# wengflow/robust-e-nerf

Measured on AMD Instinct MI355X. Metric: train_rays_per_sec, higher is better.
Workload: dtype f32; 1 GPU; BASELINE configs[1]: synthetic ficus-like event stream, 65536 events/step/GPU = 2 renders x 65536 rays x 128 samples, arch ngp, fp32, l_diff (2 renders), fwd+bwd+Adam; sampler=uniform; sampler=uniform, samples_per_ray=128, parallelism=dp1, front_prefetched=False, mlp_precision=highest, device_counts=False, device_count_overflows=0, fwd_chunks=8, dist_world_size=1

## Files before the change

include/ren_amd.h:

```cpp
#ifndef REN_AMD_H
#define REN_AMD_H

#include <stdint.h>

#ifdef __cplusplus
extern "C" {
#endif

typedef enum ren_status {
    REN_OK = 0,
    REN_ERR_BAD_ARG = -1,
    REN_ERR_UNSUPPORTED = -2,
    REN_ERR_LAUNCH = -3
} ren_status;

enum { REN_CT_AABB = 0, REN_CT_TANH = 1, REN_CT_SPHERE = 2 };

#define REN_MAX_LEVELS 16

typedef struct ren_grid_desc {
    int32_t  n_levels;
    float    scale[REN_MAX_LEVELS];
    uint32_t res[REN_MAX_LEVELS];
    uint32_t size[REN_MAX_LEVELS];
    uint32_t offset[REN_MAX_LEVELS];
    uint32_t hashed[REN_MAX_LEVELS];
} ren_grid_desc;

typedef struct ren_scene_desc {
    float   aabb[6];
    int32_t contraction_type;
} ren_scene_desc;


int ren_abi_version(void);
enum { REN_KNOB_HGB_NO_PAIRS = 0, REN_KNOB_HGB_HALVE_REGIONS = 1, REN_KNOB_MARCH_SEQUENTIAL = 2, REN_KNOB_HG_VARIANT = 3,
       REN_KNOB_VFIELD_PLAIN = 4, REN_KNOB_HGB_SUBREGION = 5, REN_KNOB_COUNT = 6 };
int ren_set_knob(int32_t knob, int32_t value);
int ren_get_knob(int32_t knob);
const char *ren_build_info(void);

int ren_trajectory_fwd(const double *ts, int64_t B, const int64_t *tab_ts, const float *tab_pos,
                       const float *tab_quat, int64_t C, float *pos, float *rot, void *stream);
int ren_raygen_fwd(const float *Kinv, const float *px, const float *pos, const float *rot,
                   int64_t B, float *rays_o, float *rays_d, void *stream);
int ren_pose_rays_fwd(const double *ts, int64_t R, const float *px, int64_t px_rows, const float *Kinv,
                      const int64_t *tab_ts, const float *tab_pos, const float *tab_quat, int64_t C,
                      float *rays_o, float *rays_d, void *stream);

int ren_ray_aabb_intersect(const float *rays_o, const float *rays_d, int64_t n_rays,
                           const float *aabb_host, float near_plane, float far_plane,
                           float *t_min, float *t_max, void *stream);
#define REN_MARCH_VERIFIED_DIV 0x100
int ren_ray_march(const float *rays_o, const float *rays_d, const float *t_min,
                  const float *t_max, const float *jitter, int64_t n_rays,
                  const float *roi_host, const int32_t *res_host, const uint8_t *binary,
                  int32_t contraction_type, float step_size, float cone_angle,
                  int32_t mode, int32_t n_uniform,
                  const int64_t *offsets, int32_t *counts,
                  int32_t *ray_indices, float *t_starts, float *t_ends, float *interval_cache,
                  int32_t cache_cap, void *stream);

int ren_march_div_check(const float *roi, int64_t *mismatches, void *stream);
int ren_uniform(uint64_t seed, uint64_t offset, int64_t n, float *out, void *stream);
int ren_exclusive_scan(const int32_t *counts, int64_t n, int64_t *offsets, int64_t *total,
                       int64_t *scratch1024 , void *stream);

int ren_count_guard(int32_t *counts, int32_t *counts_also, int64_t n_rays, const int64_t *total, int64_t capacity,
                    int64_t *n_out, int64_t *stats, void *stream);
int ren_scan_guard(int32_t *counts, int32_t *counts_also, int64_t n_rays, int64_t *offsets, int64_t *total, int64_t capacity,
                   int64_t *n_out, int64_t *stats, int64_t *scratch1024, void *stream);
int ren_frag_zero_tail(float *feat, int64_t capacity, const int64_t *n_dev, void *stream);

int ren_visibility(const int64_t *offsets, const int32_t *counts, int64_t n_rays,
                   const float *sigmas, const float *t_starts, const float *t_ends,
                   float early_stop_eps, float alpha_thre, uint8_t *keep, int32_t *kept_counts,
                   void *stream);
int ren_compact_samples(const int64_t *offsets, const int32_t *counts, const int64_t *new_offsets,
                        int64_t n_rays, const uint8_t *keep, const float *t_starts,
                        const float *t_ends, int32_t *out_ray_indices, float *out_t_starts,
                        float *out_t_ends, void *stream);
int ren_compact_features(const int64_t *offsets, const int32_t *counts, const int64_t *new_offsets, int64_t n_rays,
                         const uint8_t *keep, const float *feat_in, float *feat_out, void *stream);
int ren_pack_info(const int32_t *ray_indices, int64_t n, int64_t n_rays, int64_t *offsets,
                  int32_t *counts, void *stream);

int ren_hashgrid_fwd(const ren_grid_desc *grid, const float *table, const float *x_unit,
                     const ren_scene_desc *scene, const float *rays_o, const float *rays_d,
                     const int32_t *ray_indices, const float *t_starts, const float *t_ends,
                     int64_t n, int32_t layout, float *feat, const int64_t *n_dev, void *stream);
int ren_hashgrid_bwd(const ren_grid_desc *grid, float *grad_table, const float *x_unit,
                     const ren_scene_desc *scene, const float *rays_o, const float *rays_d,
// ... 329 lines not shown
```

robust_e_nerf_amd/_lib.py:

```python
from __future__ import annotations

import ctypes
import os
from ctypes import POINTER, Structure, c_char_p, c_double, c_float, c_int, c_int32, c_int64, c_uint32, c_void_p

HERE = os.path.dirname(os.path.abspath(__file__))
LIB_PATH = os.path.join(HERE, "csrc", "libren_amd.so")
MAX_LEVELS = 16

REN_OK, REN_ERR_BAD_ARG, REN_ERR_UNSUPPORTED, REN_ERR_LAUNCH = 0, -1, -2, -3


class RenError(RuntimeError):
    pass


class GridDesc(Structure):
    _fields_ = [("n_levels", c_int32), ("scale", c_float * MAX_LEVELS), ("res", c_uint32 * MAX_LEVELS),
                ("size", c_uint32 * MAX_LEVELS), ("offset", c_uint32 * MAX_LEVELS),
                ("hashed", c_uint32 * MAX_LEVELS)]


class SceneDesc(Structure):
    _fields_ = [("aabb", c_float * 6), ("contraction_type", c_int32)]


P = c_void_p
SIGNATURES = {
    "ren_abi_version": (c_int, []),
    "ren_build_info": (c_char_p, []),
    "ren_set_knob": (c_int, [c_int32, c_int32]),
    "ren_get_knob": (c_int, [c_int32]),
    "ren_trajectory_fwd": (c_int, [P, c_int64, P, P, P, c_int64, P, P, P]),
    "ren_raygen_fwd": (c_int, [P, P, P, P, c_int64, P, P, P]),
    "ren_pose_rays_fwd": (c_int, [P, c_int64, P, c_int64, P, P, P, P, c_int64, P, P, P]),
    "ren_ray_aabb_intersect": (c_int, [P, P, c_int64, POINTER(c_float), c_float, c_float, P, P, P]),
    "ren_march_div_check": (c_int, [POINTER(c_float), P, P]),
    "ren_ray_march": (c_int, [P, P, P, P, P, c_int64, POINTER(c_float), POINTER(c_int32), P, c_int32,
                              c_float, c_float, c_int32, c_int32, P, P, P, P, P, P, c_int32, P]),
    "ren_compact_features": (c_int, [P, P, P, c_int64, P, P, P, P]),
    "ren_uniform": (c_int, [ctypes.c_uint64, ctypes.c_uint64, c_int64, P, P]),
    "ren_exclusive_scan": (c_int, [P, c_int64, P, P, P, P]),
    "ren_count_guard": (c_int, [P, P, c_int64, P, c_int64, P, P, P]),
    "ren_scan_guard": (c_int, [P, P, c_int64, P, P, c_int64, P, P, P, P]),
    "ren_frag_zero_tail": (c_int, [P, c_int64, P, P]),
    "ren_visibility": (c_int, [P, P, c_int64, P, P, P, c_float, c_float, P, P, P]),
    "ren_compact_samples": (c_int, [P, P, P, c_int64, P, P, P, P, P, P, P]),
    "ren_pack_info": (c_int, [P, c_int64, c_int64, P, P, P]),
    "ren_hashgrid_fwd": (c_int, [POINTER(GridDesc), P, P, POINTER(SceneDesc), P, P, P, P, P, c_int64, c_int32, P, P, P]),
    "ren_hashgrid_bwd": (c_int, [POINTER(GridDesc), P, P, POINTER(SceneDesc), P, P, P, P, P, c_int64, c_int32, P, P]),
    "ren_hashgrid_bwd_input": (c_int, [POINTER(GridDesc), P, P, POINTER(SceneDesc), P, P, P, P, P, c_int64, c_int32, P, P, P]),
    "ren_hashgrid_bwd_binned_workspace_bytes": (c_int64, [c_int64]),
    "ren_hashgrid_bwd_binned": (c_int, [POINTER(GridDesc), P, P, POINTER(SceneDesc), P, P, P, P, P, c_int64, c_int32, P, P, P, P]),
    "ren_hashgrid_bwd_binned_begin": (c_int, [POINTER(GridDesc), P, POINTER(SceneDesc), P, P, P, P, P, c_int64, c_int32, P, P]),
    "ren_hashgrid_bwd_binned_scatter": (c_int, [POINTER(GridDesc), P, P, POINTER(SceneDesc), P, P, P, P, P, c_int64, c_int32, P,
                                                c_int64, c_int64, P, P]),
    "ren_hashgrid_bwd_binned_finish": (c_int, [POINTER(GridDesc), P, c_int64, c_int32, P, P]),
    "ren_mlp_fwd": (c_int, [P, c_int32, c_int32, P, POINTER(SceneDesc), P, P, P, P, P, P, P, c_int64, c_int32, P, P, P, P]),
    "ren_mlp_bwd_workspace_floats": (c_int64, [c_int32]),
    "ren_mlp_bwd": (c_int, [P, c_int32, c_int32, P, P, POINTER(SceneDesc), P, P, P, P, P, P, P, c_int64, P, P, P, P, P, P, P, P]),
    "ren_mlp_fwd_bf16": (c_int, [P, c_int32, c_int32, P, POINTER(SceneDesc), P, P, P, P, P, P, P, c_int64, c_int32, P, P, P, P]),
    "ren_mlp_bwd_bf16": (c_int, [P, c_int32, c_int32, P, P, POINTER(SceneDesc), P, P, P, P, P, P, P, c_int64, P, P, P, P, P, P, P, P]),
    "ren_mlp_act_save_floats": (c_int64, [c_int64]),
    "ren_mlp_fwd_save": (c_int, [P, c_int32, c_int32, c_int32, P, POINTER(SceneDesc), P, P, P, P, P, P, P, c_int64, P, P, P, P, P]),
    "ren_mlp_bwd_saved": (c_int, [P, c_int32, c_int32, c_int32, P, P, P, POINTER(SceneDesc), P, P, P, P, P, P, P, c_int64, P, P, P,
                                  P, P, P, P, P]),
    "ren_act_jvp_fwd": (c_int, [P, c_int32, P, c_int32, c_float, P, c_int32, c_int64, c_int32, P]),
    "ren_act_jvp_bwd": (c_int, [P, P, P, c_int32, P, c_float, P, P, c_int64, c_int32, P]),
    "ren_event_prepare": (c_int, [P, P, P, P, P, P, P, c_int64, c_float, c_float, c_double, P, P, P, P, P, P, P, P, P, P]),
    "ren_event_params_refresh": (c_int, [P, c_float, P, c_double, P, P]),
    "ren_tau_adam_step": (c_int, [P, P, P, c_double, c_double, c_double, c_double, c_double, c_int64, c_double, P]),
    "ren_event_param_grad": (c_int, [c_int32, c_int32, c_int32, P, P, P, P, P, P, P, c_int64, c_float, c_float, c_float,
                                     c_double, c_float, P, P, P, P]),
    "ren_mlp_fwd_x": (c_int, [P, c_int32, c_int32, c_int32, P, POINTER(SceneDesc), P, P, P, P, P, P, P, c_int64, c_int32, P, P, P, P, P, P]),
    "ren_mlp_bwd_x_workspace_floats": (c_int64, [c_int32]),
    "ren_mlp_bwd_x": (c_int, [P, c_int32, c_int32, c_int32, P, P, P, POINTER(SceneDesc), P, P, P, P, P, P, P, c_int64, P, P, P, P, P,
                              P, P, c_int32, P, P]),
    "ren_composite_fwd": (c_int, [P, P, c_int64, P, P, P, P, c_int32, P, P, P, P, P, P, P]),
    "ren_composite_bwd": (c_int, [P, P, c_int64, P, P, P, P, c_int32, P, P, P, P, P, P, P, P, P, P, P, P]),
    "ren_event_loss_fwd": (c_int, [P, P, P, P, c_int64, c_int32, P, P]),
    "ren_event_loss_bwd": (c_int, [P, P, P, P, c_int64, c_int32, c_float, P, P, P, P]),
    "ren_event_diff_loss_fwd": (c_int, [P, P, P, c_int32, c_float, P, c_int32, c_int64, c_int32, P, P]),
    "ren_event_diff_loss_bwd": (c_int, [P, P, P, c_int32, c_float, P, c_int32, c_int64, c_int32, c_float, P, P, P, P, P, P, P, P]),
    "ren_bkgd_param_fwd": (c_int, [P, c_int32, P, P]),
    "ren_bkgd_param_grad": (c_int, [P, c_int64, c_int32, P, P, P, P]),
# ... 109 lines not shown
```

robust_e_nerf_amd/csrc/ren_api.hip:

```cpp
#include "ren_common.h"
extern "C" int ren_abi_version(void) { return 25; }
extern "C" const char *ren_build_info(void) { return "ren_amd gfx950 (CDNA4) hipcc " __VERSION__; }

extern "C" int ren_set_knob(int32_t knob, int32_t value) {
    if (knob < 0 || knob >= REN_KNOB_COUNT) return REN_ERR_BAD_ARG;
    ren_knob_store()[knob].store(value, std::memory_order_relaxed);
    return REN_OK;
}
extern "C" int ren_get_knob(int32_t knob) { return knob < 0 || knob >= REN_KNOB_COUNT ? REN_ERR_BAD_ARG : ren_knob(knob); }
```

robust_e_nerf_amd/csrc/ren_common.h:

```cpp
#pragma once
#include <hip/hip_runtime.h>
#include <stdint.h>
#include <math.h>
#include <stdio.h>
#include "../../include/ren_amd.h"

#define REN_WAVE 64

#undef hipLaunchKernelGGL
#define hipLaunchKernelGGL(kernel, grid, block, shmem, stream, ...)            \
    do {                                                                        \
        (void)hipGetLastError();                                                \
        kernel<<<(grid), (block), (shmem), (stream)>>>(__VA_ARGS__);            \
    } while (0)

#define REN_CHECK_LAUNCH()                                   \
    do {                                                     \
        hipError_t e__ = hipGetLastError();                  \
        if (e__ != hipSuccess)                               \
            fprintf(stderr, "[ren_amd] %s:%d launch error: %s\n", __FILE__, __LINE__, hipGetErrorString(e__)); \
        return e__ == hipSuccess ? REN_OK : REN_ERR_LAUNCH;  \
    } while (0)

static inline int ren_blocks(int64_t n, int threads) { return (int)((n + threads - 1) / threads); }

#include <atomic>
#include <cstdlib>
inline std::atomic<int> *ren_knob_store() {
    static std::atomic<int> knobs[REN_KNOB_COUNT];
    static const bool init = [] {
        const char *names[REN_KNOB_COUNT] = {"REN_HGB_NO_PAIRS", "REN_HGB_HALVE_REGIONS", "REN_MARCH_SEQUENTIAL", "REN_HG_VARIANT",
                                           "REN_VFIELD_PLAIN", "REN_HGB_SUBREGION"};
        const int defaults[REN_KNOB_COUNT] = {0, 0, 0, 2, 0, 1};
        for (int k = 0; k < REN_KNOB_COUNT; ++k) {
            const char *e = getenv(names[k]);
            knobs[k].store(e ? atoi(e) : defaults[k], std::memory_order_relaxed);
        }
        return true;
    }();
    (void)init;
    return knobs;
}
static inline int ren_knob(int k) { return ren_knob_store()[k].load(std::memory_order_relaxed); }

struct ren_scene_dev {
    float lo[3], inv_ext[3];
    float hi[3];
    int ct;
};

static inline ren_scene_dev ren_make_scene(const ren_scene_desc *s) {
    ren_scene_dev d;
    for (int k = 0; k < 3; ++k) {
        d.lo[k] = s->aabb[k];
        d.hi[k] = s->aabb[3 + k];
        d.inv_ext[k] = 1.0f / (s->aabb[3 + k] - s->aabb[k]);
    }
    d.ct = s->contraction_type;
    return d;
}

__device__ __forceinline__ void ren_contract(const ren_scene_dev &sc, float x, float y, float z,
                                             float &ux, float &uy, float &uz) {
    ux = (x - sc.lo[0]) / (sc.hi[0] - sc.lo[0]);
    uy = (y - sc.lo[1]) / (sc.hi[1] - sc.lo[1]);
    uz = (z - sc.lo[2]) / (sc.hi[2] - sc.lo[2]);
    if (sc.ct == REN_CT_SPHERE) {
        ux = ux * 2.f - 1.f; uy = uy * 2.f - 1.f; uz = uz * 2.f - 1.f;
        float mag = sqrtf(ux * ux + uy * uy + uz * uz);
        if (mag > 1.f) {
            float s = (2.f - 1.f / mag) / mag;
            ux *= s; uy *= s; uz *= s;
        }
        ux = ux * 0.25f + 0.5f; uy = uy * 0.25f + 0.5f; uz = uz * 0.25f + 0.5f;
    } else if (sc.ct == REN_CT_TANH) {
        ux = (tanhf(ux - 0.5f) + 1.f) * 0.5f;
        uy = (tanhf(uy - 0.5f) + 1.f) * 0.5f;
        uz = (tanhf(uz - 0.5f) + 1.f) * 0.5f;
    }
}

__device__ __forceinline__ void ren_sample_pos(const float *__restrict__ rays_o,
                                               const float *__restrict__ rays_d,
                                               const int32_t *__restrict__ ray_indices,
                                               const float *__restrict__ t_starts,
                                               const float *__restrict__ t_ends, int64_t i,
                                               float &x, float &y, float &z, int &ray) {
    ray = ray_indices[i];
// ... 19 lines not shown
```

robust_e_nerf_amd/csrc/ren_hashgrid_binned.hip:

```cpp
#include <cstdlib>
#include "ren_hashgrid_common.h"

namespace {

constexpr int BIN_SHIFT = 13;
constexpr int BIN_ENTRIES = 1 << BIN_SHIFT;
constexpr int MAX_BINS_PER_LEVEL = 64;
constexpr int MAX_BINS = REN_MAX_LEVELS * MAX_BINS_PER_LEVEL;
#ifndef REN_SC_THREADS
#define REN_SC_THREADS 512
#endif
#ifndef REN_SC_WAVES
#define REN_SC_WAVES 6
#endif
#ifndef REN_SC_WAVES_PAIR
#define REN_SC_WAVES_PAIR 8
#endif
constexpr int SC_THREADS = REN_SC_THREADS;
constexpr int SC_ENTRIES = SC_THREADS * 8;
constexpr int CNT_THREADS = 1024, CNT_SAMPLES = 1024;
constexpr int64_t PART_ENTRIES_MIN = 1 << 16, PART_ENTRIES_MAX = 1 << 23;
constexpr int N_SUB = 8;
__device__ __forceinline__ int xcd_id() {
    unsigned x;
    asm volatile("s_getreg_b32 %0, hwreg(HW_REG_XCC_ID)" : "=s"(x));
    return (int)(x & (N_SUB - 1));
}
inline int64_t part_entries_for(int64_t n, int64_t hashed_cap) {
    int64_t p = hashed_cap;
    if (p == 0) {
        p = PART_ENTRIES_MIN;
        while (p < (1 << 21) && p * 1024 < n * 128) p <<= 1;
    }
    return p < PART_ENTRIES_MIN ? PART_ENTRIES_MIN : (p > PART_ENTRIES_MAX ? PART_ENTRIES_MAX : p);
}
constexpr int LMAX_SLOTS = 8, LMAX_STRIDE = 32;
constexpr int LMAX_WORDS = REN_MAX_LEVELS * LMAX_SLOTS * LMAX_STRIDE;

struct BinTab {
    int bin_base[REN_MAX_LEVELS + 1];
    uint32_t cap[REN_MAX_LEVELS];
    uint32_t pair[REN_MAX_LEVELS];
    uint32_t skip[REN_MAX_LEVELS];
    int sub_by_xcd;
    int cnt_stride;
    int halve;
};

struct Part {
    uint32_t gbin, single;
    uint64_t begin, end;
};

struct Workspace {
    uint32_t *counts, *level_max, *cursors, *n_parts;
    uint32_t *bin_cap;
    uint64_t *bin_start;
    Part *parts;
    char *pool;
};
constexpr int PAIR_BIN_SHIFT = 26;

struct TanSrc {
    const float *rays_do, *rays_dd, *dfeatd;
};

__device__ __forceinline__ void lds_barrier() { asm volatile("s_waitcnt lgkmcnt(0)\n\ts_barrier" ::: "memory"); }

struct SampleArgs {
    int layout;
    const float *dfeat, *x_unit;
    ren_scene_dev sc;
// ... 122 lines not shown
template <bool TAN>
__global__ __launch_bounds__(CNT_THREADS) void bin_count_kernel(GridDev g, BinTab bt, SampleArgs a,
                                                                uint32_t *__restrict__ counts) {
    __shared__ uint32_t hist[MAX_BINS];
    for (int t = threadIdx.x; t < MAX_BINS; t += CNT_THREADS) hist[t] = 0;
    __syncthreads();
    const int lane = threadIdx.x & 63;
#pragma unroll 1
    for (int k = 0; k < CNT_SAMPLES / CNT_THREADS; ++k) {
        const int64_t i = (int64_t)blockIdx.x * bt.cnt_stride * CNT_SAMPLES + k * CNT_THREADS + threadIdx.x;
        const bool inb = i < ren_eff_n(a.n, a.n_dev);
        float u[3] = {0.f, 0.f, 0.f}, ud[3];
        if (inb) unit_pos<TAN>(a, i, u, ud);
#pragma unroll 1
        for (int lvl = 0; lvl < g.n_levels; ++lvl) {
            if (bt.cap[lvl] || bt.skip[lvl]) continue;
            float d0, d1, e0, e1;
            const bool have = inb && (a.dfeat == nullptr || load_dfeat<TAN>(a, g.n_levels, lvl, i, d0, d1, e0, e1));
            const LevelPos p = level_pos(u[0], u[1], u[2], g.scale[lvl]);
            const uint32_t res = g.res[lvl], size = g.size[lvl];
            const bool hashed = g.hashed[lvl] != 0;
            bool head;
            uint32_t idx[8];
            corner_indices8(p.c[0], p.c[1], p.c[2], res, size, hashed, idx);
            const bool emit = run_tail(!hashed, have, idx[0], lane, head);
#pragma unroll
            for (int c = 0; c < 8; ++c) (void)bin_rank(!hashed, emit, idx[c] >> BIN_SHIFT, lane, hist + lvl * MAX_BINS_PER_LEVEL);
        }
    }
    __syncthreads();
    for (int t = threadIdx.x; t < MAX_BINS; t += CNT_THREADS) {
        const int lvl = t / MAX_BINS_PER_LEVEL, bin = t % MAX_BINS_PER_LEVEL;
        if (lvl < g.n_levels && bin < bt.bin_base[lvl + 1] - bt.bin_base[lvl] && hist[t])
            atomicAdd(&counts[bt.bin_base[lvl] + bin], hist[t]);
    }
}

__global__ __launch_bounds__(MAX_BINS) void bin_offsets_kernel(int n_bins, BinTab bt, uint64_t capacity_slots,
                                                               const uint32_t *__restrict__ counts,
                                                               uint32_t *__restrict__ cursors,
                                                               uint32_t *__restrict__ bin_cap,
                                                               uint64_t *__restrict__ bin_start) {
    __shared__ uint64_t s_cnt[MAX_BINS];
    const int t = threadIdx.x;
    uint64_t c = 0, slots = 0;
    bool pair = false;
    if (t < n_bins) {
        int lvl = 0;
        while (lvl + 1 < REN_MAX_LEVELS && t >= bt.bin_base[lvl + 1]) ++lvl;
        pair = bt.pair[lvl] != 0;
        c = bt.skip[lvl] ? 0 : bt.cap[lvl] ? bt.cap[lvl] : counts[t];
        if (!bt.skip[lvl] && !bt.cap[lvl] && bt.cnt_stride > 1) c = c * bt.cnt_stride + c * bt.cnt_stride / 4 + 4096;
        if (bt.halve) c = c / 2;
        c &= ~(uint64_t)7;
        if (pair) c = (c / N_SUB) & ~(uint64_t)7;
        slots = pair ? c * N_SUB : (c * 10 + 15) / 16;
        for (int x = 0; x < N_SUB; ++x) cursors[t * N_SUB + x] = 0;
    }
    s_cnt[t] = slots;
    __syncthreads();
    for (int off = 1; off < MAX_BINS; off <<= 1) {
        const uint64_t a = t >= off ? s_cnt[t - off] : 0;
        __syncthreads();
        s_cnt[t] += a;
        __syncthreads();
    }
    if (t < n_bins) {
        const uint64_t start = s_cnt[t] - slots;
        uint64_t room = start < capacity_slots ? capacity_slots - start : 0;
        if (room > slots) room = slots;
        if (room < slots) c = (pair ? room / N_SUB : room * 16 / 10) & ~(uint64_t)7;
        bin_start[t] = start < capacity_slots ? start : capacity_slots;
        bin_cap[t] = (uint32_t)c;
    }
    if (t == n_bins - 1) bin_start[n_bins] = s_cnt[t] < capacity_slots ? s_cnt[t] : capacity_slots;
}

__global__ __launch_bounds__(MAX_BINS) void bin_partition_kernel(int n_bins, uint64_t PART_ENTRIES, BinTab bt,
                                                                 const uint32_t *__restrict__ cursors,
                                                                 const uint32_t *__restrict__ bin_cap,
                                                                 Part *__restrict__ parts, uint32_t *__restrict__ n_parts) {
    __shared__ uint32_t s_np[MAX_BINS];
    const int t = threadIdx.x;
    uint64_t c = 0;
    bool pair = false;
    if (t < n_bins) {
        int lvl = 0;
        while (lvl + 1 < REN_MAX_LEVELS && t >= bt.bin_base[lvl + 1]) ++lvl;
        pair = bt.pair[lvl] != 0;
        for (int x = 0; x < (pair ? N_SUB : 1); ++x) c += cursors[t * N_SUB + x] < bin_cap[t] ? cursors[t * N_SUB + x] : bin_cap[t];
    }
    const uint32_t np = pair ? (c ? 1u : 0u) : (uint32_t)((c + PART_ENTRIES - 1) / PART_ENTRIES);
    s_np[t] = np;
    __syncthreads();
    for (int off = 1; off < MAX_BINS; off <<= 1) {
        const uint32_t b = t >= off ? s_np[t - off] : 0;
        __syncthreads();
        s_np[t] += b;
        __syncthreads();
    }
    if (t == n_bins - 1) n_parts[0] = s_np[t];
    const uint32_t pbase = s_np[t] - np;
    for (uint32_t k = 0; k < np; ++k) {
        Part p;
        p.gbin = t; p.single = np == 1;
        p.begin = (uint64_t)k * PART_ENTRIES;
        p.end = k + 1 == np ? c : p.begin + PART_ENTRIES;
        parts[pbase + k] = p;
    }
}

__device__ __forceinline__ void table_atomic(float *grad_table, uint32_t offset, uint32_t idx, float a, float b) {
    float *gt = grad_table + 2 * ((size_t)offset + idx);
    atomicAdd(gt, a);
    atomicAdd(gt + 1, b);
}

template <bool TAN, int KIND>
__global__ __launch_bounds__(SC_THREADS, KIND == 1 ? REN_SC_WAVES_PAIR : REN_SC_WAVES) void bin_scatter_kernel(
    GridDev g, BinTab bt, SampleArgs a, Workspace ws, float *__restrict__ grad_table) {
    __shared__ uint32_t hist[MAX_BINS_PER_LEVEL], loc[MAX_BINS_PER_LEVEL + 1], fit[MAX_BINS_PER_LEVEL];
    __shared__ char *gp0[MAX_BINS_PER_LEVEL], *gp1[MAX_BINS_PER_LEVEL];
    __shared__ __attribute__((aligned(16))) unsigned char stage[KIND == 1 ? SC_THREADS * 4 * 16 : SC_ENTRIES * 12];
    __shared__ float wave_max[SC_THREADS / 64];
    __shared__ int any_overflow;
    uint32_t *st_key = reinterpret_cast<uint32_t *>(stage);
    float2 *st_v = reinterpret_cast<float2 *>(stage + SC_ENTRIES * 4);
    float4 *st_p = reinterpret_cast<float4 *>(stage);
    const int64_t chunk = blockIdx.x;
    const int tid = threadIdx.x, lane = tid & 63;
    const int64_t i = chunk * SC_THREADS + tid;
    const bool inb = i < ren_eff_n(a.n, a.n_dev);
    float u[3] = {0.f, 0.f, 0.f}, ud[3] = {0.f, 0.f, 0.f};
    if (inb) unit_pos<TAN>(a, i, u, ud);
    constexpr bool pairs = KIND == 1;
    const int sub = !pairs ? 0 : bt.sub_by_xcd ? xcd_id() : (int)((chunk >> 3) & (N_SUB - 1));
#pragma unroll 1
    for (int lvl = 0; lvl < g.n_levels; ++lvl) {
        if (bt.skip[lvl]) continue;
        if (KIND == 1 && !bt.pair[lvl]) continue;
        if (KIND == 2 && bt.pair[lvl]) continue;
        if (tid < MAX_BINS_PER_LEVEL) hist[tid] = 0;
        if (tid == 0) any_overflow = 0;
        lds_barrier();
        const uint32_t res = g.res[lvl], size = g.size[lvl];
        const bool hashed = g.hashed[lvl] != 0;
        const float scale = g.scale[lvl];
        float d0 = 0.f, d1 = 0.f, e0 = 0.f, e1 = 0.f;
        const bool valid = inb && load_dfeat<TAN>(a, g.n_levels, lvl, i, d0, d1, e0, e1);
        const LevelPos p = level_pos(u[0], u[1], u[2], scale);
        const float wx1 = p.w[0], wy1 = p.w[1], wz1 = p.w[2], wx0 = 1.f - wx1, wy0 = 1.f - wy1, wz0 = 1.f - wz1;
        if (!valid) { d0 = 0.f; d1 = 0.f; e0 = 0.f; e1 = 0.f; }
        uint32_t key[8];
        float v0[8], v1[8];
        bool have;
        float vmax = 0.f;
        uint32_t idx[8];
        corner_indices8(p.c[0], p.c[1], p.c[2], res, size, hashed, idx);
        if (pairs) {
            const bool same = ((idx[0] ^ idx[1]) >> BIN_SHIFT) == 0;
#pragma unroll
            for (int j = 0; j < 4; ++j) {
                const float wyz = ((j & 1) ? wy1 : wy0) * ((j & 2) ? wz1 : wz0);
                v0[j] = wyz * d0; v1[j] = wyz * d1;
            }
            if (valid && !same) {
#pragma unroll
                for (int j = 0; j < 4; ++j) {
                    table_atomic(grad_table, g.offset[lvl], idx[2 * j], wx0 * v0[j], wx0 * v1[j]);
                    table_atomic(grad_table, g.offset[lvl], idx[2 * j + 1], wx1 * v0[j], wx1 * v1[j]);
                }
            }
            have = valid && same;
// ... 84 lines not shown
            gp0[tid] = q0; gp1[tid] = q1;
        }
        lds_barrier();
        if (have) {
            if (pairs) {
#pragma unroll
                for (int j = 0; j < 4; ++j)
                    st_p[loc[key[j] >> PAIR_BIN_SHIFT] + key[4 + j]] = make_float4(__uint_as_float(key[j]), v0[j], v1[j], wx1);
            } else {
#pragma unroll
                for (int c = 0; c < 8; ++c) {
                    const uint32_t ix = key[c] & 0x7FFFFu;
                    const uint32_t pos = loc[ix >> BIN_SHIFT] + (key[c] >> 19);
                    st_key[pos] = ix;
                    st_v[pos] = make_float2(v0[c], v1[c]);
                }
            }
        }
        lds_barrier();
        const uint32_t total = loc[MAX_BINS_PER_LEVEL];
        const bool ovf = any_overflow != 0;
        if (pairs) {
            for (uint32_t q = tid; q < total; q += SC_THREADS) {
                const float4 r = st_p[q];
                const uint32_t code = __float_as_uint(r.x), b = code >> PAIR_BIN_SHIFT;
                if (!ovf || q - loc[b] < fit[b]) {
                    reinterpret_cast<float4 *>(gp0[b])[q] = r;
                } else {
                    const uint32_t i0 = (b << BIN_SHIFT) | (code & (BIN_ENTRIES - 1));
                    const uint32_t i1 = (b << BIN_SHIFT) | ((code >> BIN_SHIFT) & (BIN_ENTRIES - 1));
                    table_atomic(grad_table, g.offset[lvl], i0, (1.f - r.w) * r.y, (1.f - r.w) * r.z);
                    table_atomic(grad_table, g.offset[lvl], i1, r.w * r.y, r.w * r.z);
                }
            }
            continue;
        }
        for (uint32_t q = tid; q < total; q += SC_THREADS) {
            const uint32_t ix = st_key[q], b = ix >> BIN_SHIFT;
            const float2 v = st_v[q];
            if (!ovf || q - loc[b] < fit[b]) {
                reinterpret_cast<uint16_t *>(gp1[b])[q] = (uint16_t)(ix & (BIN_ENTRIES - 1));
                reinterpret_cast<float2 *>(gp0[b])[q] = v;
            } else {
                table_atomic(grad_table, g.offset[lvl], ix, v.x, v.y);
            }
        }
    }
}

__device__ __forceinline__ long long to_fixed(float v, double scale) {
    return __double2ll_rn((double)v * scale);
}

__global__ __launch_bounds__(1024) void bin_accumulate_kernel(GridDev g, BinTab bt, Workspace ws,
                                                              float *__restrict__ grad_table) {
    extern __shared__ __attribute__((aligned(16))) unsigned long long acc[];
    if (blockIdx.x >= ws.n_parts[0]) return;
    const Part part = ws.parts[blockIdx.x];
    unsigned long long *acc0 = acc, *acc1 = acc + BIN_ENTRIES;
    for (int e = threadIdx.x; e < 2 * BIN_ENTRIES; e += 1024) acc[e] = 0ull;
    int lvl = 0;
    while (lvl + 1 < g.n_levels && (int)part.gbin >= bt.bin_base[lvl + 1]) ++lvl;
    int ex;
    uint32_t lmax = 0;
    for (int k = 0; k < LMAX_SLOTS; ++k) lmax = max(lmax, ws.level_max[(lvl * LMAX_SLOTS + k) * LMAX_STRIDE]);
    (void)frexpf(__uint_as_float(lmax), &ex);
    const double scale = ldexp(1.0, 38 - ex), inv_scale = ldexp(1.0, ex - 38);
    const char *base = ws.pool + ws.bin_start[part.gbin] * 16;
    const uint32_t first = ((uint32_t)part.gbin - bt.bin_base[lvl]) << BIN_SHIFT;
    const uint32_t lim = g.size[lvl] > first ? g.size[lvl] - first : 0;
    float2 *gt = reinterpret_cast<float2 *>(grad_table) + g.offset[lvl] + first;
    constexpr int FL = BIN_ENTRIES / 1024;
    float2 gv[FL];
#pragma unroll
    for (int u = 0; u < FL; ++u) {
        const uint32_t k = threadIdx.x + u * 1024;
        gv[u] = (part.single && k < lim) ? gt[k] : make_float2(0.f, 0.f);
    }
    __syncthreads();
    uint64_t e = part.begin + threadIdx.x;
    if (bt.pair[lvl]) {
        const float4 *rec = reinterpret_cast<const float4 *>(base);
        auto add = [&](const float4 &r) {
            const uint32_t code = __float_as_uint(r.x);
            const uint32_t i0 = code & (BIN_ENTRIES - 1), i1 = (code >> BIN_SHIFT) & (BIN_ENTRIES - 1);
            const float f0 = 1.f - r.w;
            atomicAdd(&acc0[i0], (unsigned long long)to_fixed(f0 * r.y, scale));
            atomicAdd(&acc1[i0], (unsigned long long)to_fixed(f0 * r.z, scale));
            atomicAdd(&acc0[i1], (unsigned long long)to_fixed(r.w * r.y, scale));
            atomicAdd(&acc1[i1], (unsigned long long)to_fixed(r.w * r.z, scale));
        };
        const uint32_t cap = ws.bin_cap[part.gbin];
        for (int x = 0; x < N_SUB; ++x) {
            const float4 *rx = rec + (size_t)x * cap;
            const uint32_t fill = ws.cursors[part.gbin * N_SUB + x];
            const uint64_t end = fill < cap ? fill : cap;
            uint64_t q = threadIdx.x;
            for (; q + 3 * 1024 < end; q += 4 * 1024) {
                float4 r[4];
#pragma unroll
                for (int u = 0; u < 4; ++u) r[u] = rx[q + u * 1024];
#pragma unroll
                for (int u = 0; u < 4; ++u) add(r[u]);
            }
            for (; q < end; q += 1024) add(rx[q]);
        }
    } else {
// ... 6 lines not shown
#pragma unroll
            for (int u = 0; u < 4; ++u) {
                atomicAdd(&acc0[ix[u]], (unsigned long long)to_fixed(v[u].x, scale));
                atomicAdd(&acc1[ix[u]], (unsigned long long)to_fixed(v[u].y, scale));
            }
        }
        for (; e < part.end; e += 1024) {
            const uint32_t idx = out_idx[e];
            const float2 v = out_v[e];
            atomicAdd(&acc0[idx], (unsigned long long)to_fixed(v.x, scale));
            atomicAdd(&acc1[idx], (unsigned long long)to_fixed(v.y, scale));
        }
    }
    __syncthreads();
#pragma unroll
    for (int u = 0; u < FL; ++u) {
        const uint32_t k = threadIdx.x + u * 1024;
        if (k >= lim) continue;
        const long long qa = (long long)acc0[k], qb = (long long)acc1[k];
        if (qa == 0 && qb == 0) continue;
        const float a = (float)((double)qa * inv_scale), b = (float)((double)qb * inv_scale);
        if (part.single) {
            float2 v = gv[u];
            v.x += a; v.y += b;
            gt[k] = v;
        } else {
            atomicAdd(&gt[k].x, a);
            atomicAdd(&gt[k].y, b);
        }
    }
}

inline size_t align256(size_t v) { return (v + 255) & ~(size_t)255; }

struct Layout { size_t counts, level_max, cursors, n_parts, bin_cap, bin_start, parts, pool, total, slots; int64_t entries, max_parts; };

Layout make_layout(int64_t n) {
    Layout L;
    const size_t E = (size_t)n * 140 + (size_t)MAX_BINS * 4096 + 16 * 8 * 16 * CNT_SAMPLES;
    L.entries = (int64_t)E;
    L.slots = (E * 10 + 15) / 16 + MAX_BINS;
    L.max_parts = (int64_t)(E / PART_ENTRIES_MIN) + MAX_BINS + 1;
    size_t o = 0;
    L.counts = o; o += MAX_BINS * 4;
    L.level_max = o; o = align256(o + LMAX_WORDS * 4);
    L.cursors = o; o = align256(o + MAX_BINS * 4 * N_SUB);
    L.n_parts = o; o = align256(o + 4);
    L.bin_cap = o; o = align256(o + MAX_BINS * 4);
    L.bin_start = o; o = align256(o + (MAX_BINS + 1) * 8);
    L.parts = o; o = align256(o + (size_t)L.max_parts * sizeof(Part));
    L.pool = o; o = align256(o + L.slots * 16);
    L.total = o;
    return L;
}

}

extern "C" int64_t ren_hashgrid_bwd_binned_workspace_bytes(int64_t n) {
    if (n < 0) return -1;
    return (int64_t)make_layout(n).total;
}

static int binned_impl(const ren_grid_desc *grid, float *grad_table, const float *x_unit,
                       const ren_scene_desc *scene, const float *rays_o, const float *rays_d,
                       const int32_t *ray_indices, const float *t_starts, const float *t_ends,
                       int64_t n, int32_t layout, const float *dfeat, void *workspace,
                       void *stream, TanSrc tan, uint32_t level_mask = 0xFFFFFFFFu, int phases = 7,
                       int64_t first = 0, int64_t m = -1, const int64_t *n_dev = nullptr) {
    GridDev g;
    int rc = make_grid(grid, g);
    if (rc) return rc;
    const bool do_begin = phases & 1, do_scatter = phases & 2, do_finish = phases & 4;
    if (m < 0) m = n - first;
    if (!workspace || n < 0 || (layout != 0 && layout != 1) || first < 0 || m < 0 || first + m > n) return REN_ERR_BAD_ARG;
    if ((do_scatter && (!dfeat || !grad_table)) || (do_finish && !grad_table)) return REN_ERR_BAD_ARG;
    if (do_scatter && phases != 7 && ((first & 31) != 0 || tan.dfeatd)) return REN_ERR_BAD_ARG;
    const bool from_rays = x_unit == nullptr;
    if ((do_begin || do_scatter) && from_rays && (!scene || !rays_o || !rays_d || !ray_indices || !t_starts || !t_ends))
        return REN_ERR_BAD_ARG;
    if (layout == 1 && g.n_levels != REN_MAX_LEVELS) return REN_ERR_UNSUPPORTED;
    if (n >= ((int64_t)1 << 28)) return REN_ERR_UNSUPPORTED;
    BinTab bt;
    int nb = 0;
    for (int l = 0; l < REN_MAX_LEVELS; ++l) {
        bt.bin_base[l] = nb;
        if (l < g.n_levels) {
            if (g.size[l] > (uint32_t)(MAX_BINS_PER_LEVEL << BIN_SHIFT)) return REN_ERR_UNSUPPORTED;
            nb += (int)((g.size[l] + BIN_ENTRIES - 1) >> BIN_SHIFT);
        }
    }
    bt.bin_base[REN_MAX_LEVELS] = nb;
    for (int l = g.n_levels; l < REN_MAX_LEVELS; ++l) bt.bin_base[l] = nb;
    int64_t hashed_cap = 0;
    const bool use_pairs = !tan.dfeatd && ren_knob(REN_KNOB_HGB_NO_PAIRS) != 1;
    for (int l = 0; l < REN_MAX_LEVELS; ++l) {
        bt.cap[l] = 0;
        bt.pair[l] = 0;
        bt.skip[l] = l < g.n_levels && !((level_mask >> l) & 1u);
        if (l < g.n_levels && g.hashed[l]) {
            const int64_t bins = (g.size[l] + BIN_ENTRIES - 1) >> BIN_SHIFT;
            bt.pair[l] = use_pairs ? 1 : 0;
            const int64_t mean = ((use_pairs ? 4 : 8) * n + bins - 1) / bins;
            bt.cap[l] = use_pairs ? (uint32_t)(N_SUB * (((mean / N_SUB + mean / 400 + 1024) + 7) & ~(int64_t)7))
                                  : (uint32_t)(mean + mean / 50 + 4096);
            if ((int64_t)bt.cap[l] > hashed_cap) hashed_cap = bt.cap[l];
        }
    }
    const int64_t part_entries = part_entries_for(n, hashed_cap);
    if (n == 0) return REN_OK;
    ren_scene_dev sc = {};
    if (scene) sc = ren_make_scene(scene);
    const Layout L = make_layout(n);
    char *w = (char *)workspace;
    Workspace ws;
    ws.counts = (uint32_t *)(w + L.counts); ws.level_max = (uint32_t *)(w + L.level_max);
    ws.cursors = (uint32_t *)(w + L.cursors);
    ws.n_parts = (uint32_t *)(w + L.n_parts); ws.bin_cap = (uint32_t *)(w + L.bin_cap);
    ws.bin_start = (uint64_t *)(w + L.bin_start);
    ws.parts = (Part *)(w + L.parts); ws.pool = w + L.pool;
    hipStream_t st = (hipStream_t)stream;
    SampleArgs a;
    a.layout = layout; a.dfeat = dfeat; a.x_unit = x_unit; a.sc = sc; a.rays_o = rays_o; a.rays_d = rays_d;
    a.ray_indices = ray_indices; a.t_starts = t_starts; a.t_ends = t_ends; a.n = n; a.tan = tan;
    a.n_dev = n_dev;
    if (n_dev && phases != 7) return REN_ERR_BAD_ARG;
    bt.halve = ren_knob(REN_KNOB_HGB_HALVE_REGIONS) == 1;
    bt.sub_by_xcd = ren_knob(REN_KNOB_HGB_SUBREGION) != 0;
    const int64_t cnt_blocks = (n + CNT_SAMPLES - 1) / CNT_SAMPLES;
    bt.cnt_stride = cnt_blocks >= 4096 ? 16 : cnt_blocks >= 2048 ? 8 : cnt_blocks >= 1024 ? 4 : 1;
    bool any_pair = false, any_single = false;
    for (int l = 0; l < g.n_levels; ++l)
        if (!bt.skip[l]) { any_pair |= bt.pair[l] != 0; any_single |= bt.pair[l] == 0; }
    if (do_begin) {
        if (hipMemsetAsync(ws.counts, 0, (MAX_BINS + LMAX_WORDS) * 4, st) != hipSuccess) return REN_ERR_LAUNCH;
        const dim3 cgrd((unsigned)((cnt_blocks + bt.cnt_stride - 1) / bt.cnt_stride)), cblk(CNT_THREADS);
        SampleArgs ac = a;
        if (phases != 7) ac.dfeat = nullptr;
        if (tan.dfeatd) hipLaunchKernelGGL(bin_count_kernel<true>, cgrd, cblk, 0, st, g, bt, ac, ws.counts);
        else            hipLaunchKernelGGL(bin_count_kernel<false>, cgrd, cblk, 0, st, g, bt, ac, ws.counts);
        hipLaunchKernelGGL(bin_offsets_kernel, dim3(1), dim3(MAX_BINS), 0, st, nb, bt, (uint64_t)L.slots, ws.counts,
                           ws.cursors, ws.bin_cap, ws.bin_start);
    }
    if (!any_pair && !any_single) return REN_OK;
    if (do_scatter && m > 0) {
        SampleArgs as = a;
        as.n = m;
        if (first) {
            if (as.x_unit) as.x_unit += 3 * first;
            if (as.ray_indices) { as.ray_indices += first; as.t_starts += first; as.t_ends += first; }
            as.dfeat += layout == 1 ? (first >> 5) * (int64_t)(REN_MAX_LEVELS * 64) : first * (int64_t)g.n_levels * 2;
        }
        const dim3 sgrd((unsigned)((m + SC_THREADS - 1) / SC_THREADS)), sblk(SC_THREADS);
        if (tan.dfeatd) hipLaunchKernelGGL((bin_scatter_kernel<true, 0>), sgrd, sblk, 0, st, g, bt, as, ws, grad_table);
        else {
            if (any_pair)   hipLaunchKernelGGL((bin_scatter_kernel<false, 1>), sgrd, sblk, 0, st, g, bt, as, ws, grad_table);
            if (any_single) hipLaunchKernelGGL((bin_scatter_kernel<false, 2>), sgrd, sblk, 0, st, g, bt, as, ws, grad_table);
        }
    }
    if (do_finish) {
        hipLaunchKernelGGL(bin_partition_kernel, dim3(1), dim3(MAX_BINS), 0, st, nb, (uint64_t)part_entries, bt, ws.cursors, ws.bin_cap, ws.parts,
                           ws.n_parts);
        const size_t acc_lds = 2 * BIN_ENTRIES * sizeof(unsigned long long);
        (void)hipFuncSetAttribute((const void *)bin_accumulate_kernel, hipFuncAttributeMaxDynamicSharedMemorySize, (int)acc_lds);
        const int64_t acc_grid = (int64_t)(L.entries / part_entries) + nb + 1;
        hipLaunchKernelGGL(bin_accumulate_kernel, dim3((unsigned)acc_grid), dim3(1024), acc_lds, st, g, bt, ws, grad_table);
    }
    REN_CHECK_LAUNCH();
}

extern "C" int ren_hashgrid_bwd_binned(const ren_grid_desc *grid, float *grad_table, const float *x_unit,
                                       const ren_scene_desc *scene, const float *rays_o, const float *rays_d,
                                       const int32_t *ray_indices, const float *t_starts, const float *t_ends,
                                       int64_t n, int32_t layout, const float *dfeat, void *workspace,
                                       const int64_t *n_dev, void *stream) {
    return binned_impl(grid, grad_table, x_unit, scene, rays_o, rays_d, ray_indices, t_starts, t_ends, n, layout,
                       dfeat, workspace, stream, TanSrc{nullptr, nullptr, nullptr}, 0xFFFFFFFFu, 7, 0, -1, n_dev);
}

extern "C" int ren_hashgrid_bwd_binned_jvp(const ren_grid_desc *grid, float *grad_table,
                                           const ren_scene_desc *scene, const float *rays_o, const float *rays_d,
                                           const float *rays_do, const float *rays_dd, const int32_t *ray_indices,
                                           const float *t_starts, const float *t_ends, int64_t n,
                                           const float *dfeat, const float *dfeatd, void *workspace, void *stream) {
    if (!rays_do || !rays_dd || !dfeatd) return REN_ERR_BAD_ARG;
    return binned_impl(grid, grad_table, nullptr, scene, rays_o, rays_d, ray_indices, t_starts, t_ends, n, 1, dfeat,
                       workspace, stream, TanSrc{rays_do, rays_dd, dfeatd});
}

extern "C" int ren_hashgrid_bwd_binned_levels(const ren_grid_desc *grid, float *grad_table, const float *x_unit,
                                              const ren_scene_desc *scene, const float *rays_o, const float *rays_d,
                                              const int32_t *ray_indices, const float *t_starts, const float *t_ends,
                                              int64_t n, int32_t layout, const float *dfeat, const float *rays_do,
                                              const float *rays_dd, const float *dfeatd, uint32_t level_mask,
                                              void *workspace, const int64_t *n_dev, void *stream) {
    if ((rays_do || rays_dd || dfeatd) && (!rays_do || !rays_dd || !dfeatd || layout != 1 || x_unit)) return REN_ERR_BAD_ARG;
    return binned_impl(grid, grad_table, x_unit, scene, rays_o, rays_d, ray_indices, t_starts, t_ends, n, layout, dfeat,
                       workspace, stream, TanSrc{rays_do, rays_dd, dfeatd}, level_mask, 7, 0, -1, n_dev);
}

extern "C" int ren_hashgrid_bwd_binned_begin(const ren_grid_desc *grid, const float *x_unit, const ren_scene_desc *scene,
                                             const float *rays_o, const float *rays_d, const int32_t *ray_indices,
                                             const float *t_starts, const float *t_ends, int64_t n, int32_t layout,
                                             void *workspace, void *stream) {
    return binned_impl(grid, nullptr, x_unit, scene, rays_o, rays_d, ray_indices, t_starts, t_ends, n, layout, nullptr,
                       workspace, stream, TanSrc{nullptr, nullptr, nullptr}, 0xFFFFFFFFu, 1);
}

extern "C" int ren_hashgrid_bwd_binned_scatter(const ren_grid_desc *grid, float *grad_table, const float *x_unit,
                                               const ren_scene_desc *scene, const float *rays_o, const float *rays_d,
                                               const int32_t *ray_indices, const float *t_starts, const float *t_ends,
                                               int64_t n, int32_t layout, const float *dfeat, int64_t first, int64_t m,
                                               void *workspace, void *stream) {
    return binned_impl(grid, grad_table, x_unit, scene, rays_o, rays_d, ray_indices, t_starts, t_ends, n, layout, dfeat,
                       workspace, stream, TanSrc{nullptr, nullptr, nullptr}, 0xFFFFFFFFu, 2, first, m);
}

extern "C" int ren_hashgrid_bwd_binned_finish(const ren_grid_desc *grid, float *grad_table, int64_t n, int32_t layout,
                                              void *workspace, void *stream) {
// ... 4 lines not shown
```

robust_e_nerf_amd/ops.py:

```python
from __future__ import annotations

import ctypes
import math
from typing import Optional, Sequence, Tuple

import torch

from . import _lib
from ._lib import GridDesc, SceneDesc, check

AABB, UN_BOUNDED_TANH, UN_BOUNDED_SPHERE = 0, 1, 2
FRAG_FLOATS_PER_BLOCK = 16 * 64
BASE_FLOATS_PER_BLOCK = 8 * 64

_DT = {torch.float32: 4, torch.float64: 8, torch.int32: 4, torch.int64: 8, torch.uint8: 1, torch.bool: 1}


KNOBS = {"hgb_no_pairs": 0, "hgb_halve_regions": 1, "march_sequential": 2, "hg_variant": 3, "vfield_plain": 4, "hgb_subregion": 5}


class knob:

    def __init__(self, name: str, value: int):
        self.k, self.v = KNOBS[name], int(value)

    def __enter__(self):
        lib = _lib.load()
        self.old = lib.ren_get_knob(self.k)
        check(lib.ren_set_knob(self.k, self.v), "ren_set_knob")

    def __exit__(self, *a):
        _lib.load().ren_set_knob(self.k, self.old)


HIDDEN_ACTS = {"softplus": 0, "relu": 1}
DENSITY_ACTS = {"shifted_trunc_exp": 0, "softplus": 1, "shifted_softplus": 2}
RADIANCE_ACTS = {"softplus": 0, "sigmoid": 1}


def activation_code(base_hidden="softplus", density="shifted_trunc_exp", head_hidden="softplus", radiance="softplus") -> int:
    try:
        return (HIDDEN_ACTS[base_hidden] | DENSITY_ACTS[density] << 2 | HIDDEN_ACTS[head_hidden] << 4 |
                RADIANCE_ACTS[radiance] << 6)
    except KeyError as e:
        raise NotImplementedError(f"activation {e.args[0]!r} (models/nerf.py:17-29)") from e


def _ptr(t: Optional[torch.Tensor], dtype=None):
    if t is None:
        return None
    if not t.is_cuda:
        raise ValueError("robust_e_nerf_amd kernels take device (ROCm) tensors; got a CPU tensor")
    if not t.is_contiguous():
        raise ValueError("tensor must be contiguous")
    if dtype is not None and t.dtype not in (dtype if isinstance(dtype, tuple) else (dtype,)):
        raise ValueError(f"expected dtype {dtype}, got {t.dtype}")
    return ctypes.c_void_p(t.data_ptr())


try:
    _raw_stream, _cur_device = torch._C._cuda_getCurrentRawStream, torch._C._cuda_getDevice
except AttributeError:
    _raw_stream = None


def _stream():
    if _raw_stream is not None:
        return ctypes.c_void_p(_raw_stream(_cur_device()))
    return ctypes.c_void_p(torch.cuda.current_stream().cuda_stream)


def _f(x):
    return ctypes.c_float(float(x))


NAN = float("nan")


def make_grid_desc(n_levels=16, n_features_per_level=2, log2_hashmap_size=19, base_resolution=16,
                   per_level_scale=1.4472692012786865, otype="HashGrid") -> Tuple[GridDesc, int]:
    import numpy as np
    if otype not in ("HashGrid", "DenseGrid", "TiledGrid"):
        raise NotImplementedError(f"pos_encoding.otype={otype}")
    if n_features_per_level != 2:
        raise NotImplementedError("n_features_per_level must be 2")
# ... 740 lines not shown
```

Measured before the change: 6.015 million rays/s.

## Add optional side-stream overlap of single-bin scatter with pair-bin accumulation

Adds an opt-in path in the binned hashgrid backward. The pair-bin scatter and its partition/accumulate run on the main stream, while the single-bin scatter runs concurrently on a per-device side stream joined by events. The final flush then handles the single bins. The path also sets a waves-per-EU occupancy hint on the accumulate kernel and rounds single-bin capacity up instead of down. Overlap is gated by a knob that defaults to off, and it adds stream/event management and a mutex on the host.

```diff
diff --git a/include/ren_amd.h b/include/ren_amd.h
--- a/include/ren_amd.h
+++ b/include/ren_amd.h
@@ -38,6 +38,8 @@
        REN_KNOB_VFIELD_PLAIN = 4, REN_KNOB_HGB_SUBREGION = 5, REN_KNOB_COUNT = 6 };
 int ren_set_knob(int32_t knob, int32_t value);
 int ren_get_knob(int32_t knob);
+int ren_hgb_overlap_set(int32_t on, int32_t min_log2);
+int ren_hgb_overlap_get(int32_t which);
 const char *ren_build_info(void);
 
 int ren_trajectory_fwd(const double *ts, int64_t B, const int64_t *tab_ts, const float *tab_pos,
diff --git a/robust_e_nerf_amd/_lib.py b/robust_e_nerf_amd/_lib.py
--- a/robust_e_nerf_amd/_lib.py
+++ b/robust_e_nerf_amd/_lib.py
@@ -31,6 +31,8 @@
     "ren_build_info": (c_char_p, []),
     "ren_set_knob": (c_int, [c_int32, c_int32]),
     "ren_get_knob": (c_int, [c_int32]),
+    "ren_hgb_overlap_set": (c_int, [c_int32, c_int32]),
+    "ren_hgb_overlap_get": (c_int, [c_int32]),
     "ren_trajectory_fwd": (c_int, [P, c_int64, P, P, P, c_int64, P, P, P]),
     "ren_raygen_fwd": (c_int, [P, P, P, P, c_int64, P, P, P]),
     "ren_pose_rays_fwd": (c_int, [P, c_int64, P, c_int64, P, P, P, P, c_int64, P, P, P]),
diff --git a/robust_e_nerf_amd/csrc/ren_api.hip b/robust_e_nerf_amd/csrc/ren_api.hip
--- a/robust_e_nerf_amd/csrc/ren_api.hip
+++ b/robust_e_nerf_amd/csrc/ren_api.hip
@@ -8,3 +8,14 @@
     return REN_OK;
 }
 extern "C" int ren_get_knob(int32_t knob) { return knob < 0 || knob >= REN_KNOB_COUNT ? REN_ERR_BAD_ARG : ren_knob(knob); }
+
+extern "C" int ren_hgb_overlap_set(int32_t on, int32_t min_log2) {
+    if (on < -1 || on > 1 || min_log2 < -1 || min_log2 > 30) return REN_ERR_BAD_ARG;
+    if (on >= 0) ren_knob_store()[REN_KNOB_HGB_OVERLAP].store(on, std::memory_order_relaxed);
+    if (min_log2 >= 0) ren_knob_store()[REN_KNOB_HGB_OVERLAP_MIN_LOG2].store(min_log2, std::memory_order_relaxed);
+    return REN_OK;
+}
+extern "C" int ren_hgb_overlap_get(int32_t which) {
+    return which == 0 ? ren_knob(REN_KNOB_HGB_OVERLAP) : which == 1 ? ren_knob(REN_KNOB_HGB_OVERLAP_MIN_LOG2)
+         : which == 2 ? ren_knob(REN_KNOB_HGB_OVERLAP_CALLS) : REN_ERR_BAD_ARG;
+}
diff --git a/robust_e_nerf_amd/csrc/ren_common.h b/robust_e_nerf_amd/csrc/ren_common.h
--- a/robust_e_nerf_amd/csrc/ren_common.h
+++ b/robust_e_nerf_amd/csrc/ren_common.h
@@ -26,14 +26,16 @@
 
 #include <atomic>
 #include <cstdlib>
+enum { REN_KNOB_HGB_OVERLAP = REN_KNOB_COUNT, REN_KNOB_HGB_OVERLAP_MIN_LOG2 = REN_KNOB_COUNT + 1,
+       REN_KNOB_HGB_OVERLAP_CALLS = REN_KNOB_COUNT + 2, REN_KNOB_SLOTS = REN_KNOB_COUNT + 3 };
 inline std::atomic<int> *ren_knob_store() {
-    static std::atomic<int> knobs[REN_KNOB_COUNT];
+    static std::atomic<int> knobs[REN_KNOB_SLOTS];
     static const bool init = [] {
-        const char *names[REN_KNOB_COUNT] = {"REN_HGB_NO_PAIRS", "REN_HGB_HALVE_REGIONS", "REN_MARCH_SEQUENTIAL", "REN_HG_VARIANT",
-                                           "REN_VFIELD_PLAIN", "REN_HGB_SUBREGION"};
-        const int defaults[REN_KNOB_COUNT] = {0, 0, 0, 2, 0, 1};
-        for (int k = 0; k < REN_KNOB_COUNT; ++k) {
-            const char *e = getenv(names[k]);
+        const char *names[REN_KNOB_SLOTS] = {"REN_HGB_NO_PAIRS", "REN_HGB_HALVE_REGIONS", "REN_MARCH_SEQUENTIAL", "REN_HG_VARIANT",
+                                           "REN_VFIELD_PLAIN", "REN_HGB_SUBREGION", "REN_HGB_OVERLAP", "REN_HGB_OVERLAP_MIN_LOG2", nullptr};
+        const int defaults[REN_KNOB_SLOTS] = {0, 0, 0, 2, 0, 1, 0, 22, 0};
+        for (int k = 0; k < REN_KNOB_SLOTS; ++k) {
+            const char *e = names[k] ? getenv(names[k]) : nullptr;
             knobs[k].store(e ? atoi(e) : defaults[k], std::memory_order_relaxed);
         }
         return true;
diff --git a/robust_e_nerf_amd/csrc/ren_hashgrid_binned.hip b/robust_e_nerf_amd/csrc/ren_hashgrid_binned.hip
--- a/robust_e_nerf_amd/csrc/ren_hashgrid_binned.hip
+++ b/robust_e_nerf_amd/csrc/ren_hashgrid_binned.hip
@@ -1,4 +1,5 @@
 #include <cstdlib>
+#include <mutex>
 #include "ren_hashgrid_common.h"
 
 namespace {
@@ -18,6 +19,7 @@
 #endif
 constexpr int SC_THREADS = REN_SC_THREADS;
 constexpr int SC_ENTRIES = SC_THREADS * 8;
+constexpr int CO_THREADS = 256;
 constexpr int CNT_THREADS = 1024, CNT_SAMPLES = 1024;
 constexpr int64_t PART_ENTRIES_MIN = 1 << 16, PART_ENTRIES_MAX = 1 << 23;
 constexpr int N_SUB = 8;
@@ -246,7 +248,7 @@
         c = bt.skip[lvl] ? 0 : bt.cap[lvl] ? bt.cap[lvl] : counts[t];
         if (!bt.skip[lvl] && !bt.cap[lvl] && bt.cnt_stride > 1) c = c * bt.cnt_stride + c * bt.cnt_stride / 4 + 4096;
         if (bt.halve) c = c / 2;
-        c &= ~(uint64_t)7;
+        c = pair ? c & ~(uint64_t)7 : (c + 7) & ~(uint64_t)7;
         if (pair) c = (c / N_SUB) & ~(uint64_t)7;
         slots = pair ? c * N_SUB : (c * 10 + 15) / 16;
         for (int x = 0; x < N_SUB; ++x) cursors[t * N_SUB + x] = 0;
@@ -270,7 +272,7 @@
     if (t == n_bins - 1) bin_start[n_bins] = s_cnt[t] < capacity_slots ? s_cnt[t] : capacity_slots;
 }
 
-__global__ __launch_bounds__(MAX_BINS) void bin_partition_kernel(int n_bins, uint64_t PART_ENTRIES, BinTab bt,
+__global__ __launch_bounds__(MAX_BINS) void bin_partition_kernel(int n_bins, int sel, uint64_t PART_ENTRIES, BinTab bt,
                                                                  const uint32_t *__restrict__ cursors,
                                                                  const uint32_t *__restrict__ bin_cap,
                                                                  Part *__restrict__ parts, uint32_t *__restrict__ n_parts) {
@@ -282,7 +284,8 @@
         int lvl = 0;
         while (lvl + 1 < REN_MAX_LEVELS && t >= bt.bin_base[lvl + 1]) ++lvl;
         pair = bt.pair[lvl] != 0;
-        for (int x = 0; x < (pair ? N_SUB : 1); ++x) c += cursors[t * N_SUB + x] < bin_cap[t] ? cursors[t * N_SUB + x] : bin_cap[t];
+        const bool selected = sel == 0 || (sel == 1) == pair;
+        for (int x = 0; selected && x < (pair ? N_SUB : 1); ++x) c += cursors[t * N_SUB + x] < bin_cap[t] ? cursors[t * N_SUB + x] : bin_cap[t];
     }
     const uint32_t np = pair ? (c ? 1u : 0u) : (uint32_t)((c + PART_ENTRIES - 1) / PART_ENTRIES);
     s_np[t] = np;
@@ -310,9 +313,10 @@
     atomicAdd(gt + 1, b);
 }
 
-template <bool TAN, int KIND>
-__global__ __launch_bounds__(SC_THREADS, KIND == 1 ? REN_SC_WAVES_PAIR : REN_SC_WAVES) void bin_scatter_kernel(
+template <bool TAN, int KIND, int THREADS = SC_THREADS>
+__global__ __launch_bounds__(THREADS, KIND == 1 ? REN_SC_WAVES_PAIR : REN_SC_WAVES) void bin_scatter_kernel(
     GridDev g, BinTab bt, SampleArgs a, Workspace ws, float *__restrict__ grad_table) {
+    constexpr int SC_THREADS = THREADS, SC_ENTRIES = THREADS * 8;
     __shared__ uint32_t hist[MAX_BINS_PER_LEVEL], loc[MAX_BINS_PER_LEVEL + 1], fit[MAX_BINS_PER_LEVEL];
     __shared__ char *gp0[MAX_BINS_PER_LEVEL], *gp1[MAX_BINS_PER_LEVEL];
     __shared__ __attribute__((aligned(16))) unsigned char stage[KIND == 1 ? SC_THREADS * 4 * 16 : SC_ENTRIES * 12];
@@ -503,7 +507,10 @@
     return __double2ll_rn((double)v * scale);
 }
 
-__global__ __launch_bounds__(1024) void bin_accumulate_kernel(GridDev g, BinTab bt, Workspace ws,
+#ifndef REN_ACC_WAVES
+#define REN_ACC_WAVES 6
+#endif
+__global__ __launch_bounds__(1024) __attribute__((amdgpu_waves_per_eu(REN_ACC_WAVES))) void bin_accumulate_kernel(GridDev g, BinTab bt, Workspace ws,
                                                               float *__restrict__ grad_table) {
     extern __shared__ __attribute__((aligned(16))) unsigned long long acc[];
     if (blockIdx.x >= ws.n_parts[0]) return;
@@ -616,6 +623,29 @@
     L.pool = o; o = align256(o + L.slots * 16);
     L.total = o;
     return L;
+}
+
+struct Fork {
+    std::mutex mu;
+    hipStream_t side = nullptr;
+    hipEvent_t forked = nullptr, joined = nullptr;
+    bool ready = false;
+};
+constexpr int MAX_DEVICES = 64;
+Fork *fork_for_current_device() {
+    static Fork forks[MAX_DEVICES];
+    int dev = -1;
+    if (hipGetDevice(&dev) != hipSuccess || dev < 0 || dev >= MAX_DEVICES) return nullptr;
+    Fork &f = forks[dev];
+    std::lock_guard<std::mutex> hold(f.mu);
+    if (!f.ready) {
+        if (hipStreamCreateWithFlags(&f.side, hipStreamNonBlocking) != hipSuccess ||
+            hipEventCreateWithFlags(&f.forked, hipEventDisableTiming) != hipSuccess ||
+            hipEventCreateWithFlags(&f.joined, hipEventDisableTiming) != hipSuccess)
+            return nullptr;
+        f.ready = true;
+    }
+    return &f;
 }
 
 }
@@ -706,28 +736,54 @@
                            ws.cursors, ws.bin_cap, ws.bin_start);
     }
     if (!any_pair && !any_single) return REN_OK;
-    if (do_scatter && m > 0) {
-        SampleArgs as = a;
-        as.n = m;
-        if (first) {
-            if (as.x_unit) as.x_unit += 3 * first;
-            if (as.ray_indices) { as.ray_indices += first; as.t_starts += first; as.t_ends += first; }
-            as.dfeat += layout == 1 ? (first >> 5) * (int64_t)(REN_MAX_LEVELS * 64) : first * (int64_t)g.n_levels * 2;
-        }
-        const dim3 sgrd((unsigned)((m + SC_THREADS - 1) / SC_THREADS)), sblk(SC_THREADS);
+    SampleArgs as = a;
+    as.n = m;
+    if (first) {
+        if (as.x_unit) as.x_unit += 3 * first;
+        if (as.ray_indices) { as.ray_indices += first; as.t_starts += first; as.t_ends += first; }
+        as.dfeat += layout == 1 ? (first >> 5) * (int64_t)(REN_MAX_LEVELS * 64) : first * (int64_t)g.n_levels * 2;
+    }
+    const dim3 sgrd((unsigned)((m + SC_THREADS - 1) / SC_THREADS)), sblk(SC_THREADS);
+    Fork *fk = nullptr;
+    bool overlap = phases == 7 && !tan.dfeatd && any_pair && any_single && m > 0 && ren_knob(REN_KNOB_HGB_OVERLAP) == 1 &&
+                   n >= ((int64_t)1 << ren_knob(REN_KNOB_HGB_OVERLAP_MIN_LOG2));
+    if (overlap) {
+        hipStreamCaptureStatus cap = hipStreamCaptureStatusNone;
+        if (hipStreamIsCapturing(st, &cap) != hipSuccess || cap != hipStreamCaptureStatusNone) { (void)hipGetLastError(); overlap = false; }
+    }
+    if (overlap && !(fk = fork_for_current_device())) return REN_ERR_LAUNCH;
+    if (overlap) ren_knob_store()[REN_KNOB_HGB_OVERLAP_CALLS].fetch_add(1, std::memory_order_relaxed);
+    if (do_scatter && m > 0 && !overlap) {
         if (tan.dfeatd) hipLaunchKernelGGL((bin_scatter_kernel<true, 0>), sgrd, sblk, 0, st, g, bt, as, ws, grad_table);
         else {
             if (any_pair)   hipLaunchKernelGGL((bin_scatter_kernel<false, 1>), sgrd, sblk, 0, st, g, bt, as, ws, grad_table);
             if (any_single) hipLaunchKernelGGL((bin_scatter_kernel<false, 2>), sgrd, sblk, 0, st, g, bt, as, ws, grad_table);
         }
     }
-    if (do_finish) {
-        hipLaunchKernelGGL(bin_partition_kernel, dim3(1), dim3(MAX_BINS), 0, st, nb, (uint64_t)part_entries, bt, ws.cursors, ws.bin_cap, ws.parts,
-                           ws.n_parts);
-        const size_t acc_lds = 2 * BIN_ENTRIES * sizeof(unsigned long long);
+    const size_t acc_lds = 2 * BIN_ENTRIES * sizeof(unsigned long long);
+    auto flush = [&](int sel, int64_t acc_grid) {
+        hipLaunchKernelGGL(bin_partition_kernel, dim3(1), dim3(MAX_BINS), 0, st, nb, sel, (uint64_t)part_entries, bt, ws.cursors, ws.bin_cap,
+                           ws.parts, ws.n_parts);
         (void)hipFuncSetAttribute((const void *)bin_accumulate_kernel, hipFuncAttributeMaxDynamicSharedMemorySize, (int)acc_lds);
-        const int64_t acc_grid = (int64_t)(L.entries / part_entries) + nb + 1;
         hipLaunchKernelGGL(bin_accumulate_kernel, dim3((unsigned)acc_grid), dim3(1024), acc_lds, st, g, bt, ws, grad_table);
+    };
+    const int64_t acc_grid_all = (int64_t)(L.entries / part_entries) + nb + 1;
+    if (overlap) {
+        std::lock_guard<std::mutex> hold(fk->mu);
+        hipLaunchKernelGGL((bin_scatter_kernel<false, 1>), sgrd, sblk, 0, st, g, bt, as, ws, grad_table);
+        if (hipEventRecord(fk->forked, st) != hipSuccess) return REN_ERR_LAUNCH;
+        int pair_bins = 0;
+        for (int l = 0; l < g.n_levels; ++l)
+            if (bt.pair[l]) pair_bins += bt.bin_base[l + 1] - bt.bin_base[l];
+        flush(1, pair_bins);
+        if (hipStreamWaitEvent(fk->side, fk->forked, 0) != hipSuccess) return REN_ERR_LAUNCH;
+        const dim3 cgrd((unsigned)((m + CO_THREADS - 1) / CO_THREADS)), cblk(CO_THREADS);
+        hipLaunchKernelGGL((bin_scatter_kernel<false, 2, CO_THREADS>), cgrd, cblk, 0, fk->side, g, bt, as, ws, grad_table);
+        if (hipEventRecord(fk->joined, fk->side) != hipSuccess || hipStreamWaitEvent(st, fk->joined, 0) != hipSuccess)
+            return REN_ERR_LAUNCH;
+        flush(2, acc_grid_all);
+    } else if (do_finish) {
+        flush(0, acc_grid_all);
     }
     REN_CHECK_LAUNCH();
 }
diff --git a/robust_e_nerf_amd/ops.py b/robust_e_nerf_amd/ops.py
--- a/robust_e_nerf_amd/ops.py
+++ b/robust_e_nerf_amd/ops.py
@@ -31,6 +31,24 @@
 
     def __exit__(self, *a):
         _lib.load().ren_set_knob(self.k, self.old)
+
+
+class hgb_overlap:
+
+    def __init__(self, on: int = -1, min_log2: int = -1):
+        self.v = (int(on), int(min_log2))
+
+    def __enter__(self):
+        lib = _lib.load()
+        self.old = (lib.ren_hgb_overlap_get(0), lib.ren_hgb_overlap_get(1))
+        check(lib.ren_hgb_overlap_set(*self.v), "ren_hgb_overlap_set")
+
+    def __exit__(self, *a):
+        _lib.load().ren_hgb_overlap_set(*self.old)
+
+
+def hgb_overlap_calls() -> int:
+    return int(_lib.load().ren_hgb_overlap_get(2))
 
 
 HIDDEN_ACTS = {"softplus": 0, "relu": 1}
```

Measured after the change: 6.042 million rays/s, median of 2. No clear change (+0.4%).
